# truongp-aws/neuronx-distributed-llama3_2

Hardware: AMD Instinct MI355X
Metric: tokens/sec (whole node) Llama-3-8B TP=8 bf16 training at 1/2/4/8 MI355X (higher is better)
Workload: dtype bf16

## Files before the change

neuronx_distributed_llama3_2_amd/csrc/flash_attn_fwd.hip:

```cpp
#include "gemm_tile.h"

#include <cstdlib>
#include <type_traits>

namespace nxd {
namespace fa {

constexpr int kBlockN = 64;

struct FwdParams {
  const uint16_t* q;
  const uint16_t* k;
  const uint16_t* v;
  uint16_t* o;
  float* lse;
  int64_t q_sb, q_ss, q_sh;
  int64_t k_sb, k_ss, k_sh;
  int64_t v_sb, v_ss, v_sh;
  int64_t o_sb, o_ss, o_sh;
  int B, Sq, Sk, Hq, Hkv;
  float scale_log2;
  int causal;
  int causal_offset;
  DropoutArgs drop;
  const int* rlo;
  const int* rhi;
};

template <int D>
__device__ __forceinline__ int swz(int row, int ch) {
  if constexpr (D == 128) {
    return ch ^ (((row & 3) << 2) | ((row >> 2) & 3));
  } else {
    return ch ^ ((((row >> 1) & 1) << 2) | ((row >> 2) & 3));
  }
}

template <int D>
__device__ __forceinline__ int lds_off(int row, int ch) {
  return row * (D * 2) + swz<D>(row, ch) * 16;
}

__device__ __forceinline__ short4_t tr_read(uint32_t a) {
  short4_t v;
  asm volatile("ds_read_b64_tr_b16 %0, %1" : "=v"(v) : "v"(a));
  return v;
}
template <int OFF>
__device__ __forceinline__ short4_t tr_read_off(uint32_t a) {
  static_assert(OFF >= 0 && OFF < 65536, "ds offset field");
  short4_t v;
  asm volatile("ds_read_b64_tr_b16 %0, %1 offset:%2" : "=v"(v) : "v"(a), "n"(OFF));
  return v;
}
template <int N>
__device__ __forceinline__ void tr_wait(short4_t (&v)[8]) {
  asm volatile("s_waitcnt lgkmcnt(%8)"
               : "+v"(v[0]), "+v"(v[1]), "+v"(v[2]), "+v"(v[3]), "+v"(v[4]), "+v"(v[5]), "+v"(v[6]), "+v"(v[7])
               : "n"(N));
}

__device__ __forceinline__ float xor32(float x, bool is_max) {
  const auto pr = __builtin_amdgcn_permlane32_swap(__float_as_uint(x), __float_as_uint(x), false, false);
  const float a = __uint_as_float(pr[0]), b = __uint_as_float(pr[1]);
  return is_max ? fmaxf(a, b) : a + b;
}

template <int D, int W, bool DROP, bool RANGE = false>
__global__ void __launch_bounds__(W * 64, 8 / W) fwd_kernel(FwdParams p) {
  constexpr int kWaves = W;
  constexpr int kBlockM = W * 32;
  constexpr int CH = D / 8;
  constexpr int KS = D / 16;
  constexpr int NDB = D / 32;
  constexpr int TILE_BYTES = kBlockN * D * 2;

  extern __shared__ __attribute__((aligned(16))) char smem[];

  const int nblk_m = (p.Sq + kBlockM - 1) / kBlockM;
  const int bh = blockIdx.x % (p.B * p.Hq);
  const int mblk = nblk_m - 1 - blockIdx.x / (p.B * p.Hq);
  const int b = bh / p.Hq;
  const int hq = bh % p.Hq;
  const int hkv = hq / (p.Hq / p.Hkv);

  const int tid = threadIdx.x, lane = tid & 63, w = tid >> 6;
  const int r = lane & 31, hh = lane >> 5;
  const int qb0 = mblk * kBlockM;
  const int q0 = qb0 + w * 32;
  const int my_q = q0 + r;

  const uint16_t* qbase = p.q + (int64_t)b * p.q_sb + (int64_t)hq * p.q_sh;
  const uint16_t* kbase = p.k + (int64_t)b * p.k_sb + (int64_t)hkv * p.k_sh;
  const uint16_t* vbase = p.v + (int64_t)b * p.v_sb + (int64_t)hkv * p.v_sh;

  bf16x8_t qf[KS];
  {
    const bool ok = my_q < p.Sq;
    const uint16_t* qrow = qbase + (int64_t)(ok ? my_q : 0) * p.q_ss;
#pragma unroll
    for (int s = 0; s < KS; ++s) {
      u32x4_t v = ok ? *reinterpret_cast<const u32x4_t*>(qrow + 16 * s + 8 * hh) : u32x4_t{0, 0, 0, 0};
      qf[s] = __builtin_bit_cast(bf16x8_t, v);
    }
  }

  int kend = p.Sk;
  if (p.causal) kend = min(p.Sk, qb0 + kBlockM + p.causal_offset);
  int tstart = 0;
  int my_lo = 0, my_hi = 0;
  int wave_lo = 0, wave_lo_max = 0, wave_hi = 0, wave_hi_min = 0;
  if constexpr (RANGE) {
    const int* rlo = p.rlo + (int64_t)b * p.Sq;
    const int* rhi = p.rhi + (int64_t)b * p.Sq;
    const int qlast = min(qb0 + kBlockM, p.Sq) - 1;
    kend = min(kend, min(rhi[qlast], p.Sk));
    tstart = min(max(rlo[qb0], 0), p.Sk) / kBlockN;
    const int qi = min(my_q, p.Sq - 1);
    my_lo = min(max(rlo[qi], 0), p.Sk);
    my_hi = min(max(rhi[qi], 0), p.Sk);
    wave_lo = __builtin_amdgcn_readlane(my_lo, 0);
    wave_lo_max = __builtin_amdgcn_readlane(my_lo, 31);
    wave_hi_min = __builtin_amdgcn_readlane(my_hi, 0);
    wave_hi = __builtin_amdgcn_readlane(my_hi, 31);
  }
  const int ntiles = kend > tstart * kBlockN ? (kend + kBlockN - 1) / kBlockN : 0;
  const int wave_qmax = q0 + 31 + p.causal_offset;
  const int wave_qmin = q0 + p.causal_offset;

  f32x16_t acc_o[NDB];
#pragma unroll
  for (int i = 0; i < NDB; ++i) acc_o[i] = f32x16_t{0};
  float m_i = -INFINITY, l_i = 0.f;
  uint32_t drow = 0;
  if constexpr (DROP) drow = drop_row_hash(p.drop.seed, b, hq + p.drop.head_offset, my_q);

  constexpr int ROWS_PER_PIECE = 1024 / (2 * D);
  constexpr int PIECES_PER_WAVE = TILE_BYTES / 1024 / kWaves;
  auto issue_tile = [&](int t, int buf) {
    char* kl = smem + buf * 2 * TILE_BYTES;
    char* vl = kl + TILE_BYTES;
#pragma unroll
    for (int i = 0; i < PIECES_PER_WAVE; ++i) {
      const int piece = w * PIECES_PER_WAVE + i;
      const int row = piece * ROWS_PER_PIECE + lane / CH;
      const int ch = swz<D>(row, lane % CH);
      const int key = min(t * kBlockN + row, p.Sk - 1);
      const uint16_t* ks = kbase + (int64_t)key * p.k_ss + ch * 8;
      const uint16_t* vs = vbase + (int64_t)key * p.v_ss + ch * 8;
      __builtin_amdgcn_global_load_lds((const __attribute__((address_space(1))) void*)ks,
                                       (__attribute__((address_space(3))) void*)(kl + piece * 1024), 16, 0, 0);
      __builtin_amdgcn_global_load_lds((const __attribute__((address_space(1))) void*)vs,
                                       (__attribute__((address_space(3))) void*)(vl + piece * 1024), 16, 0, 0);
    }
  };

  if (ntiles > 0) issue_tile(tstart, 0);
  if (kWaves == 8 && __builtin_amdgcn_readfirstlane(w) >= kWaves / 2) __builtin_amdgcn_s_setprio(1);
  __syncthreads();

  const int gi = lane & 15, tq = gi >> 2, tp = gi & 3;
  const int g = lane >> 4;
  uint32_t vlane[NDB][2];
  {
    const uint32_t s0 = lds_addr(smem);
#pragma unroll
    for (int db = 0; db < NDB; ++db) {
      const int col = 32 * db + 16 * (g & 1) + 4 * tp;
      const int ch = col >> 3, sub = (col & 7) * 2;
      vlane[db][0] = s0 + lds_off<D>(4 * hh + tq, ch) + sub;
      vlane[db][1] = s0 + lds_off<D>(4 * hh + 8 + tq, ch) + sub;
    }
  }

  auto tile = [&](int t, auto bufc) {
    constexpr int buf = decltype(bufc)::value;
    if (t + 1 < ntiles) issue_tile(t + 1, buf ^ 1);

    {
      const int kt0 = t * kBlockN;
      bool wave_active = kt0 <= wave_qmax || !p.causal;
      if constexpr (RANGE) wave_active = wave_active && kt0 < wave_hi && kt0 + kBlockN > wave_lo;
      if (wave_active) {
        const char* kl = smem + buf * 2 * TILE_BYTES;
        f32x16_t sacc[2];
        sacc[0] = f32x16_t{0};
        sacc[1] = f32x16_t{0};
        {
          u32x4_t kf[2][2];
          kf[0][0] = *reinterpret_cast<const u32x4_t*>(kl + lds_off<D>(r, hh));
          kf[0][1] = *reinterpret_cast<const u32x4_t*>(kl + lds_off<D>(32 + r, hh));
  #pragma unroll
          for (int s = 0; s < KS; ++s) {
            if (s + 1 < KS) {
              kf[(s + 1) & 1][0] = *reinterpret_cast<const u32x4_t*>(kl + lds_off<D>(r, 2 * (s + 1) + hh));
              kf[(s + 1) & 1][1] = *reinterpret_cast<const u32x4_t*>(kl + lds_off<D>(32 + r, 2 * (s + 1) + hh));
            }
            sacc[0] = __builtin_amdgcn_mfma_f32_32x32x16_bf16(__builtin_bit_cast(bf16x8_t, kf[s & 1][0]), qf[s], sacc[0], 0, 0, 0);
            sacc[1] = __builtin_amdgcn_mfma_f32_32x32x16_bf16(__builtin_bit_cast(bf16x8_t, kf[s & 1][1]), qf[s], sacc[1], 0, 0, 0);
          }
        }
        short4_t va[8], vb2[8];
          auto issue = [&](auto grpc, short4_t (&v)[8]) {
            constexpr int grp = decltype(grpc)::value;
            constexpr int OFF = buf * 2 * TILE_BYTES + TILE_BYTES + (32 * (grp >> 1) + 16 * (grp & 1)) * D * 2;
  #pragma unroll
            for (int db = 0; db < NDB; ++db) {
              v[2 * db] = tr_read_off<OFF>(vlane[db][0]);
              v[2 * db + 1] = tr_read_off<OFF>(vlane[db][1]);
            }
          };
        static_assert(NDB <= 4, "group size is 8 reads");
        issue(std::integral_constant<int, 0>{}, va);
        issue(std::integral_constant<int, 1>{}, vb2);
        bool need_mask = (kt0 + kBlockN > p.Sk) || (p.causal && kt0 + kBlockN - 1 > wave_qmin);
        if constexpr (RANGE) need_mask = need_mask || kt0 < wave_lo_max || kt0 + kBlockN > wave_hi_min;
        float tmax = -INFINITY;
        {
          if (need_mask) {
            int lim = (p.causal ? min(my_q + p.causal_offset, p.Sk - 1) : p.Sk - 1) - kt0 - 4 * hh;
            if constexpr (RANGE) lim = min(lim, my_hi - 1 - kt0 - 4 * hh);
            const int lim_lo = my_lo - kt0 - 4 * hh;
  #pragma unroll
            for (int j = 0; j < 2; ++j)
  #pragma unroll
              for (int e = 0; e < 16; ++e) {
                const int c = 32 * j + (e & 3) + 8 * (e >> 2);
                if constexpr (RANGE)
                  sacc[j][e] = (c > lim || c < lim_lo) ? -INFINITY : sacc[j][e];
                else
                  sacc[j][e] = c > lim ? -INFINITY : sacc[j][e];
              }
          }
  #pragma unroll
          for (int j = 0; j < 2; ++j)
  #pragma unroll
            for (int e = 0; e < 16; ++e) tmax = fmaxf(tmax, sacc[j][e]);
        }
        tmax = fmaxf(tmax, xor32(tmax, true)) * p.scale_log2;
        constexpr float kRescaleThreshold = 8.f;
        if (tmax > m_i + kRescaleThreshold || m_i == -INFINITY) {
          const float m_new = fmaxf(m_i, tmax);
          const float alpha = (m_i == -INFINITY) ? 0.f : __builtin_amdgcn_exp2f(m_i - m_new);
          m_i = m_new;
          l_i *= alpha;
  #pragma unroll
          for (int db = 0; db < NDB; ++db) acc_o[db] *= alpha;
        }
        const float m_use = m_i == -INFINITY ? 0.f : m_i;
        float rsum = 0.f;
        bf16x8_t pf[2][2];
  #pragma unroll
        for (int j = 0; j < 2; ++j) {
  #pragma unroll
          for (int s2 = 0; s2 < 2; ++s2) {
  #pragma unroll
            for (int e = 0; e < 8; ++e) {
              const float pv = __builtin_amdgcn_exp2f(__builtin_fmaf(sacc[j][8 * s2 + e], p.scale_log2, -m_use));
              rsum += pv;
              if constexpr (DROP) {
                const int key = kt0 + 32 * j + (e & 3) + 8 * (2 * s2 + (e >> 2)) + 4 * hh;
                pf[j][s2][e] = (__bf16)(drop_keep(drow, key, p.drop.thresh) ? pv * p.drop.scale : 0.f);
              } else {
                pf[j][s2][e] = (__bf16)pv;
              }
            }
          }
        }
        rsum = xor32(rsum, false);
        l_i += rsum;

        {
          auto mma = [&](int grp, short4_t (&v)[8]) {
            const int j = grp >> 1, s2 = grp & 1;
  #pragma unroll
            for (int db = 0; db < NDB; ++db) {
              const short4_t lo = v[2 * db], hi = v[2 * db + 1];
              const short __attribute__((ext_vector_type(8))) a8 = {lo[0], lo[1], lo[2], lo[3], hi[0], hi[1], hi[2], hi[3]};
              acc_o[db] = __builtin_amdgcn_mfma_f32_32x32x16_bf16(__builtin_bit_cast(bf16x8_t, a8), pf[j][s2], acc_o[db], 0, 0, 0);
            }
          };
          tr_wait<2 * NDB>(va);
          mma(0, va);
          issue(std::integral_constant<int, 2>{}, va);
          tr_wait<2 * NDB>(vb2);
          mma(1, vb2);
          issue(std::integral_constant<int, 3>{}, vb2);
          tr_wait<2 * NDB>(va);
          mma(2, va);
          tr_wait<0>(vb2);
          mma(3, vb2);
        }
      }
    }
    __syncthreads();
  };
  for (int t = tstart; t < ntiles; t += 2) {
    tile(t, std::integral_constant<int, 0>{});
    if (t + 1 < ntiles) tile(t + 1, std::integral_constant<int, 1>{});
  }

  if (my_q < p.Sq) {
    const float inv = l_i > 0.f ? 1.f / l_i : 0.f;
    uint16_t* orow = p.o + (int64_t)b * p.o_sb + (int64_t)my_q * p.o_ss + (int64_t)hq * p.o_sh;
#pragma unroll
    for (int db = 0; db < NDB; ++db) {
#pragma unroll
      for (int gq = 0; gq < 4; ++gq) {
        const int d = 32 * db + 8 * gq + 4 * hh;
        u32x2_t v;
        v[0] = pack2bf(acc_o[db][4 * gq + 0] * inv, acc_o[db][4 * gq + 1] * inv);
        v[1] = pack2bf(acc_o[db][4 * gq + 2] * inv, acc_o[db][4 * gq + 3] * inv);
        *reinterpret_cast<u32x2_t*>(orow + d) = v;
      }
    }
    if (hh == 0 && p.lse) {
      const float lse = l_i > 0.f ? (m_i + __log2f(l_i)) * 0.69314718055994531f : -INFINITY;
      p.lse[((int64_t)b * p.Hq + hq) * p.Sq + my_q] = lse;
    }
  }
}

}

int flash_attn_fwd_launch(const void* q, const void* k, const void* v, void* o, float* lse,
                          const int64_t* qs, const int64_t* ks, const int64_t* vs, const int64_t* os,
                          int B, int Sq, int Sk, int Hq, int Hkv, int D, float softmax_scale,
                          int causal, int causal_offset, const DropoutArgs& drop, const int* range_lo,
                          const int* range_hi, hipStream_t stream) {
  using namespace fa;
  FwdParams p{};
  p.q = (const uint16_t*)q;
  p.k = (const uint16_t*)k;
  p.v = (const uint16_t*)v;
  p.o = (uint16_t*)o;
  p.lse = lse;
  p.q_sb = qs[0]; p.q_ss = qs[1]; p.q_sh = qs[2];
  p.k_sb = ks[0]; p.k_ss = ks[1]; p.k_sh = ks[2];
  p.v_sb = vs[0]; p.v_ss = vs[1]; p.v_sh = vs[2];
  p.o_sb = os[0]; p.o_ss = os[1]; p.o_sh = os[2];
  p.B = B; p.Sq = Sq; p.Sk = Sk; p.Hq = Hq; p.Hkv = Hkv;
  p.scale_log2 = softmax_scale * 1.4426950408889634f;
  p.causal = causal;
  p.causal_offset = causal_offset;
  p.drop = drop;
  p.rlo = range_lo;
  p.rhi = range_hi;
  const bool range = range_lo != nullptr;
  if (range && (range_hi == nullptr || drop.enabled())) return -3;
  if (Hkv <= 0 || Hq % Hkv != 0) return -1;
  if (D != 128 && D != 64) return -2;
  const bool w8 = ((Sq + 255) / 256) * B * Hq >= 512;
  const int rows = w8 ? 256 : 128;
  const int grid = ((Sq + rows - 1) / rows) * B * Hq;
  if (grid == 0) return 0;
  const size_t lds = 2 * 2 * kBlockN * D * 2;
#define NXD_FA_LAUNCH(DD, WW, DR, ...) \
  hipLaunchKernelGGL((fwd_kernel<DD, WW, DR, ##__VA_ARGS__>), dim3(grid), dim3(WW * 64), lds, stream, p)
  if (range) {
    if (D == 128) {
      if (w8) NXD_FA_LAUNCH(128, 8, false, true); else NXD_FA_LAUNCH(128, 4, false, true);
    } else {
      if (w8) NXD_FA_LAUNCH(64, 8, false, true); else NXD_FA_LAUNCH(64, 4, false, true);
    }
  } else if (drop.enabled()) {
    if (D == 128) {
      if (w8) NXD_FA_LAUNCH(128, 8, true); else NXD_FA_LAUNCH(128, 4, true);
    } else {
      if (w8) NXD_FA_LAUNCH(64, 8, true); else NXD_FA_LAUNCH(64, 4, true);
    }
  } else if (D == 128) {
    if (w8) NXD_FA_LAUNCH(128, 8, false); else NXD_FA_LAUNCH(128, 4, false);
  } else {
    if (w8) NXD_FA_LAUNCH(64, 8, false); else NXD_FA_LAUNCH(64, 4, false);
  }
#undef NXD_FA_LAUNCH
  return (int)hipGetLastError();
}

}
```

Measured before the change: 21850.

## Deepen K prefetch, interleave softmax exp with PV MFMAs, stage output via LDS

The QK^T loop now prefetches K fragments up to four slices ahead, using inline ds_read_b128 with explicit lgkmcnt waits and sched barriers. The softmax exponent and bf16 packing for each P group is sliced and interleaved between the PV MFMAs of the previous group, so transcendental work overlaps the matrix core. The output epilogue repacks accumulators with permlane32_swap into per-wave LDS staging and writes 16-byte coalesced rows to global memory, replacing the scattered 8-byte stores. These changes add register pressure from the deeper prefetch and depend on hand-counted waitcnts and LDS reuse after the main loop.

```diff
diff --git a/neuronx_distributed_llama3_2_amd/csrc/flash_attn_fwd.hip b/neuronx_distributed_llama3_2_amd/csrc/flash_attn_fwd.hip
--- a/neuronx_distributed_llama3_2_amd/csrc/flash_attn_fwd.hip
+++ b/neuronx_distributed_llama3_2_amd/csrc/flash_attn_fwd.hip
@@ -7,6 +7,7 @@
 namespace fa {
 
 constexpr int kBlockN = 64;
+constexpr int kKDepth = 4;
 
 struct FwdParams {
   const uint16_t* q;
@@ -60,6 +61,18 @@
                : "n"(N));
 }
 
+template <int OFF>
+__device__ __forceinline__ u32x4_t k_read_off(uint32_t a) {
+  static_assert(OFF >= 0 && OFF < 65536, "ds offset field");
+  u32x4_t v;
+  asm volatile("ds_read_b128 %0, %1 offset:%2" : "=v"(v) : "v"(a), "n"(OFF));
+  return v;
+}
+template <int N>
+__device__ __forceinline__ void k_wait(u32x4_t (&v)[2]) {
+  asm volatile("s_waitcnt lgkmcnt(%2)" : "+v"(v[0]), "+v"(v[1]) : "n"(N));
+}
+
 __device__ __forceinline__ float xor32(float x, bool is_max) {
   const auto pr = __builtin_amdgcn_permlane32_swap(__float_as_uint(x), __float_as_uint(x), false, false);
   const float a = __uint_as_float(pr[0]), b = __uint_as_float(pr[1]);
@@ -173,6 +186,10 @@
     }
   }
 
+  uint32_t klane[KS];
+#pragma unroll
+  for (int s = 0; s < KS; ++s) klane[s] = lds_addr(smem) + lds_off<D>(r, 2 * s + hh);
+
   auto tile = [&](int t, auto bufc) {
     constexpr int buf = decltype(bufc)::value;
     if (t + 1 < ntiles) issue_tile(t + 1, buf ^ 1);
@@ -182,22 +199,33 @@
       bool wave_active = kt0 <= wave_qmax || !p.causal;
       if constexpr (RANGE) wave_active = wave_active && kt0 < wave_hi && kt0 + kBlockN > wave_lo;
       if (wave_active) {
-        const char* kl = smem + buf * 2 * TILE_BYTES;
         f32x16_t sacc[2];
         sacc[0] = f32x16_t{0};
         sacc[1] = f32x16_t{0};
         {
-          u32x4_t kf[2][2];
-          kf[0][0] = *reinterpret_cast<const u32x4_t*>(kl + lds_off<D>(r, hh));
-          kf[0][1] = *reinterpret_cast<const u32x4_t*>(kl + lds_off<D>(32 + r, hh));
+          constexpr int P = KS < kKDepth ? KS : kKDepth;
+          constexpr int OFF0 = buf * 2 * TILE_BYTES, OFF1 = OFF0 + 32 * D * 2;
+          u32x4_t kf[P][2];
+  #pragma unroll
+          for (int s = 0; s < P; ++s) {
+            kf[s][0] = k_read_off<OFF0>(klane[s]);
+            kf[s][1] = k_read_off<OFF1>(klane[s]);
+          }
   #pragma unroll
           for (int s = 0; s < KS; ++s) {
-            if (s + 1 < KS) {
-              kf[(s + 1) & 1][0] = *reinterpret_cast<const u32x4_t*>(kl + lds_off<D>(r, 2 * (s + 1) + hh));
-              kf[(s + 1) & 1][1] = *reinterpret_cast<const u32x4_t*>(kl + lds_off<D>(32 + r, 2 * (s + 1) + hh));
+            const int ahead = (s + P - 1 < KS ? s + P - 1 : KS - 1) - s;
+            u32x4_t(&f)[2] = kf[s % P];
+            if (ahead == 3) k_wait<6>(f);
+            else if (ahead == 2) k_wait<4>(f);
+            else if (ahead == 1) k_wait<2>(f);
+            else k_wait<0>(f);
+            sacc[0] = __builtin_amdgcn_mfma_f32_32x32x16_bf16(__builtin_bit_cast(bf16x8_t, f[0]), qf[s], sacc[0], 0, 0, 0);
+            sacc[1] = __builtin_amdgcn_mfma_f32_32x32x16_bf16(__builtin_bit_cast(bf16x8_t, f[1]), qf[s], sacc[1], 0, 0, 0);
+            if (s + P < KS) {
+              f[0] = k_read_off<OFF0>(klane[s + P]);
+              f[1] = k_read_off<OFF1>(klane[s + P]);
             }
-            sacc[0] = __builtin_amdgcn_mfma_f32_32x32x16_bf16(__builtin_bit_cast(bf16x8_t, kf[s & 1][0]), qf[s], sacc[0], 0, 0, 0);
-            sacc[1] = __builtin_amdgcn_mfma_f32_32x32x16_bf16(__builtin_bit_cast(bf16x8_t, kf[s & 1][1]), qf[s], sacc[1], 0, 0, 0);
+            __builtin_amdgcn_sched_barrier(0);
           }
         }
         short4_t va[8], vb2[8];
@@ -249,48 +277,51 @@
         }
         const float m_use = m_i == -INFINITY ? 0.f : m_i;
         float rsum = 0.f;
-        bf16x8_t pf[2][2];
-  #pragma unroll
-        for (int j = 0; j < 2; ++j) {
-  #pragma unroll
-          for (int s2 = 0; s2 < 2; ++s2) {
-  #pragma unroll
-            for (int e = 0; e < 8; ++e) {
-              const float pv = __builtin_amdgcn_exp2f(__builtin_fmaf(sacc[j][8 * s2 + e], p.scale_log2, -m_use));
-              rsum += pv;
-              if constexpr (DROP) {
-                const int key = kt0 + 32 * j + (e & 3) + 8 * (2 * s2 + (e >> 2)) + 4 * hh;
-                pf[j][s2][e] = (__bf16)(drop_keep(drow, key, p.drop.thresh) ? pv * p.drop.scale : 0.f);
-              } else {
-                pf[j][s2][e] = (__bf16)pv;
-              }
+        bf16x8_t pf[4];
+        auto slice = [&](int grp, int e0, int e1) {
+          const int j = grp >> 1, s2 = grp & 1;
+  #pragma unroll
+          for (int e = e0; e < e1; ++e) {
+            const float pv = __builtin_amdgcn_exp2f(__builtin_fmaf(sacc[j][8 * s2 + e], p.scale_log2, -m_use));
+            rsum += pv;
+            if constexpr (DROP) {
+              const int key = kt0 + 32 * j + (e & 3) + 8 * (2 * s2 + (e >> 2)) + 4 * hh;
+              pf[grp][e] = (__bf16)(drop_keep(drow, key, p.drop.thresh) ? pv * p.drop.scale : 0.f);
+            } else {
+              pf[grp][e] = (__bf16)pv;
             }
           }
-        }
+        };
+        constexpr bool kPin = !DROP;
+        auto group = [&](auto grpc, short4_t (&v)[8]) {
+          constexpr int grp = decltype(grpc)::value;
+          if constexpr (kPin) __builtin_amdgcn_sched_barrier(0);
+  #pragma unroll
+          for (int db = 0; db < NDB; ++db) {
+            const short4_t lo = v[2 * db], hi = v[2 * db + 1];
+            const short __attribute__((ext_vector_type(8))) a8 = {lo[0], lo[1], lo[2], lo[3], hi[0], hi[1], hi[2], hi[3]};
+            acc_o[db] = __builtin_amdgcn_mfma_f32_32x32x16_bf16(__builtin_bit_cast(bf16x8_t, a8), pf[grp], acc_o[db], 0, 0, 0);
+            if constexpr (kPin && grp < 3) {
+              slice(grp + 1, db * (8 / NDB), (db + 1) * (8 / NDB));
+              __builtin_amdgcn_sched_barrier(0);
+            }
+          }
+          if constexpr (!kPin && grp < 3) slice(grp + 1, 0, 8);
+        };
+
+        slice(0, 0, 8);
+        tr_wait<2 * NDB>(va);
+        group(std::integral_constant<int, 0>{}, va);
+        issue(std::integral_constant<int, 2>{}, va);
+        tr_wait<2 * NDB>(vb2);
+        group(std::integral_constant<int, 1>{}, vb2);
+        issue(std::integral_constant<int, 3>{}, vb2);
+        tr_wait<2 * NDB>(va);
+        group(std::integral_constant<int, 2>{}, va);
+        tr_wait<0>(vb2);
+        group(std::integral_constant<int, 3>{}, vb2);
         rsum = xor32(rsum, false);
         l_i += rsum;
-
-        {
-          auto mma = [&](int grp, short4_t (&v)[8]) {
-            const int j = grp >> 1, s2 = grp & 1;
-  #pragma unroll
-            for (int db = 0; db < NDB; ++db) {
-              const short4_t lo = v[2 * db], hi = v[2 * db + 1];
-              const short __attribute__((ext_vector_type(8))) a8 = {lo[0], lo[1], lo[2], lo[3], hi[0], hi[1], hi[2], hi[3]};
-              acc_o[db] = __builtin_amdgcn_mfma_f32_32x32x16_bf16(__builtin_bit_cast(bf16x8_t, a8), pf[j][s2], acc_o[db], 0, 0, 0);
-            }
-          };
-          tr_wait<2 * NDB>(va);
-          mma(0, va);
-          issue(std::integral_constant<int, 2>{}, va);
-          tr_wait<2 * NDB>(vb2);
-          mma(1, vb2);
-          issue(std::integral_constant<int, 3>{}, vb2);
-          tr_wait<2 * NDB>(va);
-          mma(2, va);
-          tr_wait<0>(vb2);
-          mma(3, vb2);
-        }
       }
     }
     __syncthreads();
@@ -300,21 +331,33 @@
     if (t + 1 < ntiles) tile(t + 1, std::integral_constant<int, 1>{});
   }
 
-  if (my_q < p.Sq) {
+  {
     const float inv = l_i > 0.f ? 1.f / l_i : 0.f;
-    uint16_t* orow = p.o + (int64_t)b * p.o_sb + (int64_t)my_q * p.o_ss + (int64_t)hq * p.o_sh;
-#pragma unroll
-    for (int db = 0; db < NDB; ++db) {
-#pragma unroll
-      for (int gq = 0; gq < 4; ++gq) {
-        const int d = 32 * db + 8 * gq + 4 * hh;
-        u32x2_t v;
-        v[0] = pack2bf(acc_o[db][4 * gq + 0] * inv, acc_o[db][4 * gq + 1] * inv);
-        v[1] = pack2bf(acc_o[db][4 * gq + 2] * inv, acc_o[db][4 * gq + 3] * inv);
-        *reinterpret_cast<u32x2_t*>(orow + d) = v;
+    {
+      char* st = smem + w * (32 * D * 2);
+#pragma unroll
+      for (int db = 0; db < NDB; ++db) {
+#pragma unroll
+        for (int k = 0; k < 2; ++k) {
+          const f32x16_t& a = acc_o[db];
+          const uint32_t x0 = pack2bf(a[8 * k + 0] * inv, a[8 * k + 1] * inv), x1 = pack2bf(a[8 * k + 2] * inv, a[8 * k + 3] * inv);
+          const uint32_t y0 = pack2bf(a[8 * k + 4] * inv, a[8 * k + 5] * inv), y1 = pack2bf(a[8 * k + 6] * inv, a[8 * k + 7] * inv);
+          const auto p0 = __builtin_amdgcn_permlane32_swap(x0, y0, false, false);
+          const auto p1 = __builtin_amdgcn_permlane32_swap(x1, y1, false, false);
+          *reinterpret_cast<u32x4_t*>(st + lds_off<D>(r, 4 * db + 2 * k + hh)) = u32x4_t{p0[0], p1[0], p0[1], p1[1]};
+        }
       }
-    }
-    if (hh == 0 && p.lse) {
+      asm volatile("s_waitcnt lgkmcnt(0)" ::: "memory");
+      uint16_t* ob = p.o + (int64_t)b * p.o_sb + (int64_t)hq * p.o_sh;
+      constexpr int RPI = 64 / CH;
+#pragma unroll
+      for (int i = 0; i < 32 / RPI; ++i) {
+        const int row = i * RPI + lane / CH, c = lane % CH;
+        const u32x4_t v = *reinterpret_cast<const u32x4_t*>(st + lds_off<D>(row, c));
+        if (q0 + row < p.Sq) *reinterpret_cast<u32x4_t*>(ob + (int64_t)(q0 + row) * p.o_ss + c * 8) = v;
+      }
+    }
+    if (my_q < p.Sq && hh == 0 && p.lse) {
       const float lse = l_i > 0.f ? (m_i + __log2f(l_i)) * 0.69314718055994531f : -INFINITY;
       p.lse[((int64_t)b * p.Hq + hq) * p.Sq + my_q] = lse;
     }
```

Result: no change. 21720 (-0.6%).
